# gunrock/mini

Measured on AMD Instinct MI355X. Metric: MTEPS (million traversed edges/sec) BFS advance+filter, RMAT-22, higher is better.
Workload: dtype int32

## Files before the change

### include/mgx/bfs_fused.hpp

```cpp
#pragma once
#include <cstdlib>
#include <cstring>
#include <memory>

#include "runtime.hpp"
#include "env.hpp"
#include "wave.hpp"

namespace mgx {

constexpr int BFS_MAX_TRACE = 4096;
constexpr int BFS_VSHIFT = 38;
constexpr u64 BFS_EMASK = (1ull << BFS_VSHIFT) - 1ull;

struct bfs_ctrl_t {
  u64 cursor[3];
  u64 pad_a_[13];
  u64 lcursor[3];
  u64 pad_b_[13];
  u64 ledges[3];
  u64 pad_c_[13];
  u64 reached;
  u64 pad_d_[15];
  u64 merged_new;
// ... 41 lines not shown

struct bfs_fused_args_t {
  const u32* row_offsets;
  const int* col_indices;
  int* labels;
  u32* visited;
  unsigned char* mark;
  u32* frontier_bits;
  u32* fr_row[2];
  u32* fr_off[2];
  u32* lq_row[2];
  u32* lq_off[2];
  bfs_ctrl_t* ctrl;
  const u32* in_offsets;
  const int* in_indices;
  const int* old_of_new;
  const int* new_of_old;
  int long_min;
  u32 hot_min_edges;
  int mode;
  float alpha;
  int n;
  int count_marks;
  const int* ub_col;
  const u32* ub_col24;
  const int* ub_owner;
  u32 ub_units;
  u32 ub_units_pad;
  u32 ub_hot_only;
  const u32* ubf_col24;
  const int* ubf_owner;
  u32 ubf_units_pad;
  u32 dense_div;
  u32 vs_v[4];
  u32 vs_v9;
  u32 vs_edges;
  u32 vs_div;
  u32 vs_dummy;
  u32* flush_buf;
  u32 defer_min_marks;
  u32 defer_words;
  u32 defer_reach_mul, defer_reach_div;
  int lazy_pull;
  int merged_pull;
  u32 chain_max_edges;
  u32 chain_big_edges;
  u32 lazy_div;
  u32* slot_marks;
  const int* cold_owner;
  const int* cold_dst;
  int cold_slices;
  u32 cold_lo[BFS_COLD_MAX_SLICES];
  u32 cold_off[BFS_COLD_MAX_SLICES + 1];
  u32 cold_wgs[BFS_COLD_MAX_SLICES + 1];
  u32* cold_flush;
  u32 cold_all = 0;
  u64 cold_all_pairs = 0;
  const u32* cold_pk = nullptr;
  const u32* cold_cbase = nullptr;
  u64 cold_pk_mask = 0;
  u32 cold_ranks = 1;
  u32 cold_cb[BFS_COLD_MAX_SLICES + 1] = {};
  u32* d2_list = nullptr;
  u32 d2_list_cap = 0;
  u32* d2_newbits = nullptr;
  u32* d2_front = nullptr;
  const int* vs_col = nullptr;
  const int* colds_owner = nullptr;
  const int* colds_dst = nullptr;
  u32 colds_off[BFS_COLD_MAX_SLICES + 1] = {};
#ifdef MGX_LAB
  int flags;
  int build_diag;
  int dense_diag;
#endif
};

#ifdef MGX_LAB
#define MGX_LAB_GET(obj, field, product_value) ((obj).field)
#else
#define MGX_LAB_GET(obj, field, product_value) (product_value)
#endif

template <int NT, int WORDS>
__device__ __forceinline__ void bfs_copy_prefix(u32* __restrict__ dst, const u32* __restrict__ src) {
  static_assert(WORDS % 4 == 0, "whole 16-byte pieces");
  constexpr int Q = WORDS / 4;
  constexpr int IT = (Q + NT - 1) / NT;
  const uint4* const s4 = (const uint4*)src;
  uint4* const d4 = (uint4*)dst;
  uint4 v[IT];
#pragma unroll
  for (int k = 0; k < IT; ++k) {
    const int i = k * NT + (int)threadIdx.x;
    v[k] = s4[i < Q ? i : Q - 1];
  }
#pragma unroll
  for (int k = 0; k < IT; ++k) {
    const int i = k * NT + (int)threadIdx.x;
    if (i < Q) d4[i] = v[k];
  }
}

constexpr int BFS_COLD_WGS = 64;
constexpr int BFS_COLD_WGS_MAX = 1024;
constexpr int BFS_COLD_WORDS = 20384;

constexpr int BFS_MARK_CTRS = 8;
constexpr int BFS_MARK_STRIDE = 32;

__device__ __forceinline__ void bfs_body_finish(const bfs_fused_args_t& a, int marks, int slot, int stat_level, int* s_int) {
  if (!a.slot_marks && !a.count_marks) return;
  marks = wave_sum(marks);
  if ((threadIdx.x & (WAVE - 1)) == 0 && marks) atomicAdd(&s_int[0], marks);
  __syncthreads();
  if (threadIdx.x == 0 && s_int[0]) {
    if (a.slot_marks) atomicAdd(&a.slot_marks[((slot & 1) * BFS_MARK_CTRS + (int)(blockIdx.x % BFS_MARK_CTRS)) * BFS_MARK_STRIDE], (u32)s_int[0]);
    if (a.count_marks) {
      atomicAdd(&a.ctrl->claims, (u64)s_int[0]);
      if (stat_level < 64) atomicAdd(&a.ctrl->claims_level[stat_level], (u64)s_int[0]);
    }
  }
}
__device__ __forceinline__ void bfs_slot_marks_clear(const bfs_fused_args_t& a, int slot) {
  if (a.slot_marks)
    for (int i = 0; i < BFS_MARK_CTRS; ++i) a.slot_marks[((slot & 1) * BFS_MARK_CTRS + i) * BFS_MARK_STRIDE] = 0u;
}

__device__ __forceinline__ void bfs_ctrl_reset(bfs_ctrl_t* c) {
  for (int i = 0; i < 3; ++i) { c->cursor[i] = 0; c->lcursor[i] = 0; c->ledges[i] = 0; }
  c->merged_new = 0;
  c->sum_edges = c->sum_frontier = c->sum_long_edges = c->sum_long_vertices = 0;
  c->reached = 1;
  c->claims = 0;
  for (int i = 0; i < 64; ++i) c->claims_level[i] = 0;
  c->pull_edges = 0;
  c->done = c->levels = c->pull = c->push_levels = 0;
  c->d2_append_level = c->d2_declared_level = -1;
  c->small_levels = c->slots = 0;
  c->dist_done = c->dist_levels = 0;
  for (int i = 0; i < 4; ++i) { c->slot_level[i] = 0; c->skip_build[i] = 0; }
  c->flush_count[0] = c->flush_count[1] = 0;
  c->fb_slot = 0;
  c->dense_slots = 0;
  c->vshort_slots = 0;
  c->lazy_slot = -1;
  c->lazy_slots = 0;
  c->cold_slot = -1;
  c->cold_slots = 0;
  c->mini_slots = 0;
  for (int i = 0; i < 4; ++i) c->mini_blocks[i] = 0u;
  c->reached_mini = 0;
  c->d2_frozen_level = -1;
  for (int i = 0; i < 16; ++i) ((u32*)c->d2_level_kind)[i] = 0u;
  for (int i = 0; i < 64; ++i) c->d2_level_new[i] = 0u;
  c->sssp_thr = 0x7f7fffffu;
  c->sssp_far_cnt[0] = c->sssp_far_cnt[1] = 0;
  c->sssp_far_min[0] = c->sssp_far_min[1] = 0x7f7fffffu;
  for (int i = 0; i < 64; ++i) c->stamp[i] = 0;
}

__host__ __device__ __forceinline__ u32 bfs_lq_pad(u32 deg) { return (deg + 63u) & ~63u; }
__host__ __device__ __forceinline__ u32 bfs_lq_degree(u32 entry, u32 next_entry) {
  return ((next_entry & ~63u) - (entry & ~63u)) - ((64u - (entry & 63u)) & 63u);
}

__device__ __forceinline__ void bfs_seed_queue(const bfs_fused_args_t& a, u32 row) {
  bfs_ctrl_t* c = a.ctrl;
  const u32 ro = a.row_offsets[row];
  const u32 deg = a.row_offsets[row + 1] - ro;
  const bool is_long = a.long_min > 0 && deg >= (u32)a.long_min;
  (is_long ? a.lq_row : a.fr_row)[0][0] = ro;
  (is_long ? a.lq_off : a.fr_off)[0][0] = is_long ? (deg & 63u) : 0u;
  (is_long ? c->lcursor : c->cursor)[0] = deg ? ((1ull << BFS_VSHIFT) | (u64)(is_long ? bfs_lq_pad(deg) : deg)) : 0ull;
  if (is_long) c->ledges[0] = deg;
}

template <int NT>
__device__ __forceinline__ void bfs_init_body(const bfs_fused_args_t& a, int src, long long nwords, const bfs_ctrl_t* prev_ctrl,
                                              bfs_ctrl_t* prev_head, int head_words, u32 blk, u32 nblk) {
  if (prev_head && blk == 0) {
    const u32* const from = (const u32*)prev_ctrl;
    u32* const to = (u32*)prev_head;
    for (int i = threadIdx.x; i < head_words; i += NT) to[i] = from[i];
    __syncthreads();
  }
  const int src_old = src;
  if (a.new_of_old) src = a.new_of_old[src];
  const long long tid = (long long)blk * NT + threadIdx.x;
  const long long nth = (long long)nblk * NT;
  const long long n = a.n;
  for (long long i = tid; i < (n + 3) / 4; i += nth) {
    if (i * 4 + 4 <= n) {
      const long long j = i * 4;
      const int4 l = make_int4(src_old == j ? 0 : -1, src_old == j + 1 ? 0 : -1, src_old == j + 2 ? 0 : -1,
                               src_old == j + 3 ? 0 : -1);
      *(int4*)(a.labels + j) = l;
      *(u32*)(a.mark + i * 4) = 0u;
    } else {
      for (long long j = i * 4; j < n; ++j) { a.labels[j] = (j == src_old) ? 0 : -1; a.mark[j] = 0; }
    }
  }
  const u32 src_bit = 1u << (src & 31);
  for (long long w = tid; w < nwords; w += nth) {
    const u32 seed = (w == (src >> 5)) ? src_bit : 0u;
    a.visited[w] = seed;
    a.frontier_bits[w] = seed;
  }
  if (tid == 0) {
    bfs_ctrl_reset(a.ctrl);
    bfs_slot_marks_clear(a, 0);
    bfs_slot_marks_clear(a, 1);
    bfs_seed_queue(a, (u32)src);
  }
}
__global__ __launch_bounds__(BLOCK) void k_bfs_fused_init(bfs_fused_args_t a, int src, long long nwords, const bfs_ctrl_t* prev_ctrl,
                                                          bfs_ctrl_t* prev_head, int head_words) {
  bfs_init_body<BLOCK>(a, src, nwords, prev_ctrl, prev_head, head_words, blockIdx.x, gridDim.x);
}

__device__ __forceinline__ bool bfs_open_level(const bfs_fused_args_t& a, int level, int slot) {
  bfs_ctrl_t* const c = a.ctrl;
  const u64 cur = c->cursor[slot % 3];
  const u64 lcur = c->lcursor[slot % 3];
  const long long nf = (long long)(cur >> BFS_VSHIFT) + (long long)(lcur >> BFS_VSHIFT);
  const u64 long_edges = c->ledges[slot % 3];
  const u64 E = (cur & BFS_EMASK) + long_edges;
  c->cursor[(slot + 2) % 3] = 0;
  c->lcursor[(slot + 2) % 3] = 0;
  c->ledges[(slot + 2) % 3] = 0;
  if (level < 64) c->stamp[level] = __builtin_amdgcn_s_memrealtime();
  if (nf == 0) {
    if (!c->done) { c->done = 1; c->levels = level; }
    return false;
  }
  if (level < BFS_MAX_TRACE) c->trace[level] = ((u64)nf << BFS_VSHIFT) | E;
  c->sum_edges += E;
  c->sum_frontier += (u64)nf;
  c->sum_long_edges += long_edges;
  c->sum_long_vertices += lcur >> BFS_VSHIFT;
  if (a.mode == 1 && !c->pull) {
    const float unvisited = (float)((long long)a.n - (long long)c->reached);
    if (unvisited < (float)nf * a.alpha) c->pull = 1;
  }
  if (!c->pull) c->push_levels += 1;
  return true;
}

__device__ __forceinline__ bool bfs_level_pulls(const bfs_fused_args_t& a, const bfs_ctrl_t* c, int slot) {
  if (a.mode != 1) return false;
  if (c->pull) return true;
  const long long nf = (long long)(c->cursor[slot % 3] >> BFS_VSHIFT) + (long long)(c->lcursor[slot % 3] >> BFS_VSHIFT);
  const float unvisited = (float)((long long)a.n - (long long)c->reached);
  return unvisited < (float)nf * a.alpha;
}

__device__ __forceinline__ void bfs_begin_level(const bfs_fused_args_t& a, int level, int partitioned) {
  bfs_ctrl_t* const c = a.ctrl;
  if (partitioned && level > 0 && c->merged_new == 0 && !c->dist_done) { c->dist_done = 1; c->dist_levels = level; }
  (void)bfs_open_level(a, level, level);
}
__global__ void k_bfs_level_begin(bfs_fused_args_t a, int level, int partitioned) {
  if (blockIdx.x != 0 || threadIdx.x != 0) return;
  bfs_begin_level(a, level, partitioned);
}

__device__ __forceinline__ bool bfs_d2_frozen(const bfs_ctrl_t* c, int level) {
  const int f = c->d2_frozen_level;
  return f >= 0 && level > f;
}

__device__ __forceinline__ void bfs_resolve(const bfs_ctrl_t* c, int arg, int& slot, int& level) {
  if (arg >= 0) { slot = level = arg; return; }
  slot = -1 - arg;
  level = c->slot_level[slot & 3];
}
__host__ __device__ __forceinline__ int bfs_slot_arg(int slot) { return -1 - slot; }

constexpr int BFS_FLUSH_WORDS = 20352;
constexpr int BFS_FLUSH_MAX = 1024;
constexpr int BFS_FLUSH_RUNS = BFS_FLUSH_WORDS / 32;

__device__ __forceinline__ u32 bfs_defer_limit(const bfs_fused_args_t& a, u32 hot_n) {
  if (!a.flush_buf || hot_n == 0u) return 0u;
  const u32 range = hot_n < a.defer_words * 32u ? hot_n : a.defer_words * 32u;
  return a.ctrl->reached * (u64)a.defer_reach_mul < (u64)range * (u64)a.defer_reach_div ? range : 0u;
}

template <int NT>
__device__ __forceinline__ int bfs_hot_epilogue(const bfs_fused_args_t& a, const u32* hot, u32 defer_words, int slot,
                                                int* s_red, int marks) {
  if (defer_words == 0u) return 0;
  constexpr int PERT = (BFS_FLUSH_WORDS + NT - 1) / NT;
  if (threadIdx.x == 0) { s_red[0] = 0; s_red[1] = -1; }
  __syncthreads();
  const int wm = wave_sum(marks);
  if (lane_id() == 0 && wm) atomicAdd(&s_red[0], wm);
  __syncthreads();
  const int total = s_red[0];
  if (total == 0) return 0;
  if (MGX_LAB_GET(a, dense_diag, 0) & 8) return total;
  if ((u32)total > a.defer_min_marks) {
    if (threadIdx.x == 0) {
      const u32 k = atomicAdd(&a.ctrl->flush_count[slot & 1], 1u);
      s_red[1] = k < (u32)BFS_FLUSH_MAX ? (int)k : -1;
    }
    __syncthreads();
    const int k = s_red[1];
    if (k >= 0) {
      u32* const out = a.flush_buf + (size_t)k * BFS_FLUSH_WORDS;
#pragma unroll
      for (int q = 0; q < PERT; ++q) {
        const u32 i = (u32)q * NT + threadIdx.x;
        if (i < a.defer_words) out[i] = i < defer_words ? hot[i] : 0u;
      }
      return total;
    }
  }
  constexpr int CH = 5;
#pragma unroll
  for (int q0 = 0; q0 < PERT; q0 += CH) {
    u32 vis[CH];
#pragma unroll
    for (int k = 0; k < CH; ++k) {
      const u32 i = (u32)(q0 + k) * NT + threadIdx.x;
      vis[k] = __hip_atomic_load(a.visited + (i < defer_words ? i : 0u), __ATOMIC_RELAXED, __HIP_MEMORY_SCOPE_WAVEFRONT);
    }
#pragma unroll
    for (int k = 0; k < CH; ++k) {
      if (q0 + k >= PERT) break;
      const u32 i = (u32)(q0 + k) * NT + threadIdx.x;
      u32 w = i < defer_words ? (hot[i] & ~vis[k]) : 0u;
      const u32 base = i * 32u;
      while (w) {
        const int b = __ffs((int)w) - 1;
        w &= w - 1u;
        a.mark[base + (u32)b] = 1;
      }
    }
  }
  return total;
}

struct __attribute__((aligned(4))) bfs_u32x2 { u32 x, y; };

constexpr int BFS_BUILD_NT = 1024;
constexpr int BFS_BUILD_VPB = 16 * BFS_BUILD_NT;
constexpr int BFS_BUILD_LIST = 8 * BFS_BUILD_NT;

inline int bfs_build_grid(long long n_local, int nt = BFS_BUILD_NT) { return (int)((n_local + 16 * nt - 1) / (16 * nt)); }

template <int NT, bool FROM_MARKS>
__global__ __launch_bounds__(NT, NT == 512 ? 4 : 4) void k_bfs_build(bfs_fused_args_t a, int arg, const u32* __restrict__ bits,
                                                  int* __restrict__ labels, int n_local, int ranks, int rank,
                                                  int stop_when_done) {
  constexpr int NW = NT / WAVE;
  constexpr int LIST = 8 * NT;
  constexpr int PER = LIST / NT;
  constexpr u64 CNT1 = 1ull << 40;
  constexpr u64 DEGMASK = CNT1 - 1ull;
  __shared__ u32 st_v[LIST];
  __shared__ u32 st_d[LIST];
  __shared__ u64 s_scan[NW + 1];
  __shared__ u64 s_base[2];
  __shared__ u32 s_long_edges;
  bfs_ctrl_t* const c = a.ctrl;
  int slot, level;
  bfs_resolve(c, arg, slot, level);
  if (stop_when_done && c->done) return;
  if (!FROM_MARKS && bfs_d2_frozen(c, level)) return;
  if (arg < 0 && c->skip_build[slot & 3]) return;
  if (FROM_MARKS && blockIdx.x == 0 && threadIdx.x == 0) c->fb_slot = slot + 1;
  const long long i0 = (((long long)blockIdx.x + (long long)(threadIdx.x >> 6) * gridDim.x) * 64 + (threadIdx.x & 63)) * 16;
  const int new_label = level + 1;
  const int* __restrict__ old_of_new = a.old_of_new;
  const u32 long_min = a.long_min > 0 ? (u32)a.long_min : 0xFFFFFFFFu;

  u32 flushed16 = 0;
  if (FROM_MARKS && a.flush_buf) {
    const u32 F = (MGX_LAB_GET(a, build_diag, 0) & 32) ? 0u : c->flush_count[slot & 1];
    if (F) {
      __shared__ u32 s_or[NW][WAVE];
      const int wave = threadIdx.x >> 6, lane = threadIdx.x & 63;
      for (int hr = 0; hr < NW; ++hr) {
        const long long run = (long long)blockIdx.x + (long long)hr * gridDim.x;
        if (run >= (long long)(a.defer_words / 32u)) break;
        const unsigned short* const col = (const unsigned short*)a.flush_buf + run * 64 + lane;
        u32 acc = 0;
#pragma unroll 16
        for (u32 k = (u32)wave; k < F; k += NW) acc |= col[(size_t)k * (BFS_FLUSH_WORDS * 2)];
        s_or[wave][lane] = acc;
        __syncthreads();
        if (wave == hr) {
#pragma unroll
          for (int w = 0; w < NW; ++w) flushed16 |= s_or[w][lane];
        }
        __syncthreads();
      }
    }
  }

  u32 new16 = 0;
  if (i0 < n_local) {
    const u32 valid = (n_local - i0 >= 16) ? 0xFFFFu : ((1u << (int)(n_local - i0)) - 1u);
    if (FROM_MARKS) {
      const uint4 m = *(const uint4*)(a.mark + i0);
      const u32 x[4] = {m.x, m.y, m.z, m.w};
      u32 m16 = 0;
#pragma unroll
      for (int q = 0; q < 4; ++q) m16 |= (((x[q] & 0x01010101u) * 0x10204080u) >> 28) << (4 * q);
      m16 |= flushed16;
      unsigned short* const vis16 = (unsigned short*)a.visited + (i0 >> 4);
      const u32 old16 = *vis16;
      new16 = m16 & ~old16 & valid;
      if (new16) *vis16 = (unsigned short)(old16 | new16);
      ((unsigned short*)a.frontier_bits)[i0 >> 4] = (unsigned short)new16;
    } else {
      for (int q = 0; q < 16; ++q) {
        const long long v = (i0 + q) * ranks + rank;
        if (((valid >> q) & 1u) && ((bits[v >> 5] >> (v & 31)) & 1u)) new16 |= 1u << q;
      }
    }
  }
  u64 total64;
  const u64 before = block_exclusive_sum_lean<NW>((u64)__popc(new16), s_scan, &total64);
  const int total = (int)total64;
  if (total == 0) return;
  if (threadIdx.x == 0) atomicAdd(&c->reached, (u64)total);

  u64* const cur_s = &c->cursor[(slot + 1) % 3];
  u64* const cur_l = &c->lcursor[(slot + 1) % 3];
  u32* __restrict__ const out_row_s = a.fr_row[(slot + 1) & 1];
  u32* __restrict__ const out_off_s = a.fr_off[(slot + 1) & 1];
  u32* __restrict__ const out_row_l = a.lq_row[(slot + 1) & 1];
  u32* __restrict__ const out_off_l = a.lq_off[(slot + 1) & 1];

  for (int first = 0; first < total; first += LIST) {
    {
      u32 rest = new16;
      int at = (int)before - first;
      while (rest) {
        const int q = __ffs((int)rest) - 1;
        rest &= rest - 1;
        if (at >= 0 && at < LIST) st_v[at] = (u32)(i0 + q);
        ++at;
      }
    }
    if (threadIdx.x == 0) s_long_edges = 0;
    __syncthreads();
    const int cnt = (total - first < LIST) ? total - first : LIST;
#pragma unroll
    for (int q = 0; q < PER; ++q) {
      const int i = q * NT + threadIdx.x;
      if (i < cnt) {
        const u32 v = st_v[i];
        bfs_u32x2 ext;
        if (MGX_LAB_GET(a, build_diag, 0) & 2) { ext.x = v * 8u; ext.y = v * 8u + 3u; }
        else ext = *(const bfs_u32x2*)(a.row_offsets + v);
        if (!(MGX_LAB_GET(a, build_diag, 0) & 1)) labels[old_of_new ? old_of_new[v] : (int)v] = new_label;
        st_v[i] = ext.x;
        st_d[i] = ext.y - ext.x;
      }
    }
    __syncthreads();
    u32 ro[PER], dg[PER];
#pragma unroll
    for (int q = 0; q < PER; ++q) {
      const int i = threadIdx.x * PER + q;
      ro[q] = (i < cnt) ? st_v[i] : 0u;
      dg[q] = (i < cnt) ? st_d[i] : 0u;
    }
    u64 loc[PER];
    u64 sum_s = 0, sum_l = 0;
    u32 longmask = 0, long_true = 0;
#pragma unroll
    for (int q = 0; q < PER; ++q) {
      const u32 deg = dg[q];
      const bool is_long = deg >= long_min;
      if (is_long) { longmask |= 1u << q; long_true += deg; }
      loc[q] = is_long ? sum_l : sum_s;
      const u64 add = deg ? (CNT1 | (u64)(is_long ? bfs_lq_pad(deg) : deg)) : 0ull;
      if (is_long) sum_l += add; else sum_s += add;
    }
    long_true = wave_sum(long_true);
    if ((threadIdx.x & (WAVE - 1)) == 0 && long_true) atomicAdd(&s_long_edges, long_true);
    u64 tot_s, tot_l;
    const u64 ex_s = block_exclusive_sum_lean<NW>(sum_s, s_scan, &tot_s);
    const u64 ex_l = block_exclusive_sum_lean<NW>(sum_l, s_scan, &tot_l);
    if (threadIdx.x == 0) {
      if (MGX_LAB_GET(a, build_diag, 0) & 4) { s_base[0] = ((u64)blockIdx.x * 4096) << BFS_VSHIFT; s_base[1] = ((u64)blockIdx.x * 4096) << BFS_VSHIFT; }
      else {
      s_base[0] = (tot_s >> 40) ? atomicAdd(cur_s, ((tot_s >> 40) << BFS_VSHIFT) | (tot_s & DEGMASK)) : 0ull;
      s_base[1] = (tot_l >> 40) ? atomicAdd(cur_l, ((tot_l >> 40) << BFS_VSHIFT) | (tot_l & DEGMASK)) : 0ull;
      }
      if (tot_l >> 40) atomicAdd(&c->ledges[(slot + 1) % 3], (u64)s_long_edges);
    }
    __syncthreads();
#pragma unroll
    for (int q = 0; q < PER; ++q) {
      if (dg[q] != 0u) {
        const bool is_long = (longmask >> q) & 1u;
        const u64 base = is_long ? s_base[1] : s_base[0];
        const u64 at = (is_long ? ex_l : ex_s) + loc[q];
        const u64 slot = (base >> BFS_VSHIFT) + (at >> 40);
        (is_long ? out_row_l : out_row_s)[slot] = ro[q];
        (is_long ? out_off_l : out_off_s)[slot] =
            (u32)((base & BFS_EMASK) + (at & DEGMASK)) | (is_long ? (dg[q] & 63u) : 0u);
      }
    }
    __syncthreads();
  }
}

__device__ __forceinline__ bool bfs_build_is_lazy(const bfs_fused_args_t& a, int slot) {
  if (a.lazy_div == 0u || !a.slot_marks) return false;
  u64 M = 0;
#pragma unroll
  for (int i = 0; i < BFS_MARK_CTRS; ++i) M += a.slot_marks[((slot & 1) * BFS_MARK_CTRS + i) * BFS_MARK_STRIDE];
  return M * (u64)a.lazy_div >= (u64)(u32)a.n;
}

struct bfs_d2_fuse_t {
  const u32* maps = nullptr;
  int nmaps = 0;
  long long stride = 0;
  long long nwords = 0;
  u32* merged = nullptr;
  u32* clear = nullptr;
  u32* list_head = nullptr;
};
template <int NT, int DIST = 0, int RANKS = 1>
__global__ __launch_bounds__(NT, 4) void k_bfs_build2(bfs_fused_args_t a, int arg, int* __restrict__ labels, int n,
                                                      const u32* __restrict__ bits = nullptr, int ranks = 1, int rank = 0,
                                                      bfs_d2_fuse_t fz = bfs_d2_fuse_t()) {
  constexpr int NW = NT / WAVE;
  constexpr u64 CNT1 = 1ull << 40;
  constexpr u64 DEGMASK = CNT1 - 1ull;
  __shared__ u64 s_scan[NW + 1];
  __shared__ u64 s_base[2];
  __shared__ u32 s_long_edges;
  __shared__ u32 s_or[NW][WAVE];
  bfs_ctrl_t* const c = a.ctrl;
  uint4 pre_m = make_uint4(0u, 0u, 0u, 0u);
  u32 pre_old16 = 0u;
  if (!DIST) {
    const long long j0 = ((((long long)blockIdx.x + (long long)(threadIdx.x % NW) * gridDim.x) * 64 + (threadIdx.x / NW)) * 16);
    const long long jc = j0 < (long long)n ? j0 : 0;
    pre_m = *(const uint4*)(a.mark + jc);
    pre_old16 = ((const unsigned short*)a.visited)[jc >> 4];
  }
  int slot, level;
  bfs_resolve(c, arg, slot, level);
  if (!DIST && (c->done || c->skip_build[slot & 3])) return;
  if (DIST && bfs_d2_frozen(c, level)) return;
  if (DIST == 2 && fz.list_head && blockIdx.x == 0 && threadIdx.x == 0) fz.list_head[0] = 0u;
  const bool lazy = !DIST && (bfs_build_is_lazy(a, slot) || (a.lazy_pull && c->pull));
  if (!DIST && blockIdx.x == 0 && threadIdx.x == 0) {
    c->fb_slot = slot + 1;
    c->lazy_slot = lazy ? slot + 1 : -1;
    if (lazy) c->lazy_slots += 1;
  }
  const int wave = threadIdx.x >> 6, lane = threadIdx.x & 63;
  const int my_run = threadIdx.x % NW, my_group = threadIdx.x / NW;
  const long long i0 = (((long long)blockIdx.x + (long long)my_run * gridDim.x) * 64 + my_group) * 16;
  const int new_label = level + 1;
  const u32 long_min = a.long_min > 0 ? (u32)a.long_min : 0xFFFFFFFFu;

  u32 flushed16 = 0;
  if (!DIST && a.flush_buf) {
    const u32 F = (MGX_LAB_GET(a, build_diag, 0) & 32) ? 0u : c->flush_count[slot & 1];
    if (F) {
      for (int hr = 0; hr < NW; ++hr) {
        const long long run = (long long)blockIdx.x + (long long)hr * gridDim.x;
        if (run >= (long long)(a.defer_words / 32u)) break;
        const uint4* const base = (const uint4*)(a.flush_buf + (size_t)run * 32) + (lane & 7);
        uint4 acc = make_uint4(0u, 0u, 0u, 0u);
#pragma unroll 8
        for (u32 k = (u32)wave * 8u + ((u32)lane >> 3); k < F; k += 8u * NW) {
          const uint4 v = base[(size_t)k * (BFS_FLUSH_WORDS / 4)];
          acc.x |= v.x; acc.y |= v.y; acc.z |= v.z; acc.w |= v.w;
        }
#pragma unroll
        for (int sh = 8; sh < 64; sh <<= 1) {
          acc.x |= __shfl_xor(acc.x, sh, WAVE); acc.y |= __shfl_xor(acc.y, sh, WAVE);
          acc.z |= __shfl_xor(acc.z, sh, WAVE); acc.w |= __shfl_xor(acc.w, sh, WAVE);
        }
        if (lane < 8) *(uint4*)(&s_or[wave][lane * 4]) = acc;
        __syncthreads();
        if (my_run == hr) {
#pragma unroll
          for (int w = 0; w < NW; ++w) flushed16 |= (u32)((const unsigned short*)&s_or[w][0])[my_group];
        }
        __syncthreads();
      }
    }
  }

  if (!DIST && a.cold_dst && c->cold_slot == slot && !(MGX_LAB_GET(a, build_diag, 0) & 64)) {
    static_assert(NW == 8, "one wave per run");
    u32* const s_run = &s_or[0][0];
    const long long run = (long long)blockIdx.x + (long long)wave * gridDim.x;
    const long long v0 = run * 1024;
    int sl = -1;
    for (int q = 0; q < a.cold_slices; ++q)
      if (v0 >= (long long)a.cold_lo[q] && v0 < (long long)a.cold_lo[q] + (long long)BFS_COLD_WORDS * 32) sl = q;
    uint4 acc = make_uint4(0u, 0u, 0u, 0u);
    if (sl >= 0) {
      const u32 rel = (u32)((v0 - (long long)a.cold_lo[sl]) >> 10);
// ... 413 lines not shown
```

### include/mgx/bfs_fused_chain.hpp

```cpp
#pragma once
#include "bfs_fused.hpp"

namespace mgx {

constexpr int BFS_CHAIN_NT = 1024;
constexpr int BFS_CHAIN_CAP = 6144;
constexpr int BFS_CHAIN_EPT = 4;
constexpr int BFS_CHAIN_CAP_BIG = 12288;
constexpr size_t bfs_chain_lds_bytes(int cap = BFS_CHAIN_CAP) {
  return (size_t)(BFS_CHAIN_NT / 64 + 2) * 8 + (size_t)(3 * cap + 4) * 4 + 64;
}

constexpr u32 BFS_CHAIN_EARLY_EDGES = 1536;
__device__ __forceinline__ bool bfs_rule_pulls(const bfs_fused_args_t& a, u64 reached, u64 nf) {
  const float unvisited = (float)((long long)a.n - (long long)reached);
  return unvisited < (float)(long long)nf * a.alpha;
}
__device__ __forceinline__ u32 bfs_chain_edge_limit(const bfs_fused_args_t& a, u64 reached, u32 max_edges) {
  const bool late = reached * 4ull >= (u64)(u32)a.n;
  return late || max_edges < BFS_CHAIN_EARLY_EDGES ? max_edges : BFS_CHAIN_EARLY_EDGES;
}
__device__ __forceinline__ bool bfs_level_is_chained(const bfs_fused_args_t& a, u64 cur, u64 lcur, u64 ledges, u32 max_edges, int list_cap = BFS_CHAIN_CAP) {
  if (max_edges == 0u) return false;
  const u64 nf = (cur >> BFS_VSHIFT) + (lcur >> BFS_VSHIFT);
  const u64 E = (cur & BFS_EMASK) + ledges;
  if (a.mode == 1 && (a.ctrl->pull || bfs_rule_pulls(a, a.ctrl->reached, nf))) return false;
  const u32 lim = bfs_chain_edge_limit(a, a.ctrl->reached, max_edges);
  const u64 cap = lim < (u32)list_cap ? lim : (u32)list_cap;
  return nf <= (u64)list_cap && E <= cap;
}
__device__ __forceinline__ bool bfs_level_is_chained(const bfs_fused_args_t& a, u64 cur, u64 lcur, u64 ledges) {
  return bfs_level_is_chained(a, cur, lcur, ledges, a.chain_max_edges);
}

template <int NT, bool INPLACE = false, int CAP = BFS_CHAIN_CAP>
__device__ __forceinline__ void bfs_chain_body(const bfs_fused_args_t& a, int slot, int level) {
  constexpr int NW = NT / WAVE;
  constexpr int EPT = BFS_CHAIN_EPT;
  constexpr u64 CNT1 = 1ull << 40;
  constexpr u64 DEGMASK = CNT1 - 1ull;
  static_assert(CAP % NT == 0, "chain list shape");
  extern __shared__ __attribute__((aligned(16))) char smem[];
  u64* const s_scan = (u64*)smem;
  u32* const s_off = (u32*)(s_scan + NW + 2);
  u32* const s_row = s_off + CAP + 2;
  u32* const s_win = s_row + CAP;
  int* const s_i = (int*)(s_win + CAP);
  bfs_ctrl_t* const c = a.ctrl;
  const int lane = lane_id();
  const u32 long_min = a.long_min > 0 ? (u32)a.long_min : 0xFFFFFFFFu;
  const u32 lim_e = INPLACE ? a.chain_big_edges : a.chain_max_edges;

  int nf;
  u32 E;
  {
    const u64 cur = c->cursor[slot % 3], lcur = c->lcursor[slot % 3];
    const int nf_l = (int)(lcur >> BFS_VSHIFT), nf_s = (int)(cur >> BFS_VSHIFT);
    const u32 El = (u32)(lcur & BFS_EMASK), Es = (u32)(cur & BFS_EMASK);
    const u32* __restrict__ lq_row = a.lq_row[slot & 1];
    const u32* __restrict__ lq_off = a.lq_off[slot & 1];
    const u32* __restrict__ fr_row = a.fr_row[slot & 1];
    const u32* __restrict__ fr_off = a.fr_off[slot & 1];
    nf = nf_l + nf_s;
    u64 run = 0;
    for (int first = 0; first < nf; first += NT) {
      const int i = first + threadIdx.x;
      u32 row = 0, deg = 0;
      if (i < nf_l) {
        const u32 e0 = lq_off[i], e1 = (i + 1 < nf_l) ? lq_off[i + 1] : El;
        row = lq_row[i];
        deg = bfs_lq_degree(e0, e1);
      } else if (i < nf) {
        const int j = i - nf_l;
        const u32 e0 = fr_off[j], e1 = (j + 1 < nf_s) ? fr_off[j + 1] : Es;
        row = fr_row[j];
        deg = e1 - e0;
      }
      u64 tot;
      const u64 ex = run + block_exclusive_sum_lean<NW>((u64)deg, s_scan, &tot);
      if (i < nf) { s_row[i] = row; s_off[i] = (u32)ex; }
      run += tot;
    }
    E = (u32)run;
    if (threadIdx.x == 0) s_off[nf] = E;
  }

  for (int chained = 0;; ++chained) {
    if (threadIdx.x == 0) {
      if (level < 64) c->stamp[level] = __builtin_amdgcn_s_memrealtime();
      if (level < BFS_MAX_TRACE) c->trace[level] = ((u64)nf << BFS_VSHIFT) | (u64)E;
      c->sum_edges += (u64)E;
      c->sum_frontier += (u64)nf;
      c->push_levels += 1;
      c->small_levels += 1;
      if (chained == 0 && !INPLACE) c->slots += 1;
      s_i[0] = 0;
    }
    __syncthreads();

    {
      int top = 1;
      while (top * 2 < nf) top *= 2;
      for (u32 base = 0; base < E; base += NT * EPT) {
        u32 r[EPT];
        int sj[EPT];
        bool act[EPT];
#pragma unroll
        for (int k = 0; k < EPT; ++k) {
          r[k] = base + (u32)(k * NT) + threadIdx.x;
          act[k] = r[k] < E;
          if (!act[k]) r[k] = 0;
          sj[k] = 0;
        }
        if (nf > 1)
          for (int step = top; step > 0; step >>= 1) {
#pragma unroll
            for (int k = 0; k < EPT; ++k) {
              const int j = sj[k] + step;
              if (j < nf && s_off[j] <= r[k]) sj[k] = j;
            }
          }
        int d[EPT];
#pragma unroll
        for (int k = 0; k < EPT; ++k) d[k] = a.col_indices[act[k] ? s_row[sj[k]] + (r[k] - s_off[sj[k]]) : 0u];
        u32 seen[EPT];
#pragma unroll
        for (int k = 0; k < EPT; ++k) seen[k] = act[k] ? a.visited[(u32)d[k] >> 5] : 0xFFFFFFFFu;
        u32 old[EPT];
#pragma unroll
        for (int k = 0; k < EPT; ++k) {
          const u32 bit = 1u << (d[k] & 31);
          old[k] = (seen[k] & bit) ? 0xFFFFFFFFu : atomicOr(a.visited + ((u32)d[k] >> 5), bit);
        }
#pragma unroll
        for (int k = 0; k < EPT; ++k) {
          const bool win = !(old[k] & (1u << (d[k] & 31)));
          const u64 bal = __ballot(win);
          if (bal) {
            int at = 0;
            if (lane == 0) at = atomicAdd(&s_i[0], __popcll(bal));
            at = __builtin_amdgcn_readfirstlane(at);
            if (win) s_win[at + rank_in_mask(bal)] = (u32)d[k];
          }
        }
      }
    }
    __syncthreads();

    const int W = s_i[0];
    const int new_label = level + 1;
    u64 run = 0;
    constexpr int WPT = 4;
    for (int first = 0; first < W; first += WPT * NT) {
      u32 ro[WPT], dg[WPT];
      u64 mine = 0;
#pragma unroll
      for (int q = 0; q < WPT; ++q) {
        const int i = first + threadIdx.x * WPT + q;
        ro[q] = 0; dg[q] = 0;
        if (i < W) {
          const u32 v = s_win[i];
          const bfs_u32x2 ext = *(const bfs_u32x2*)(a.row_offsets + v);
          ro[q] = ext.x;
          dg[q] = ext.y - ext.x;
          a.labels[a.old_of_new ? a.old_of_new[v] : (int)v] = new_label;
        }
        if (dg[q]) mine += CNT1 | (u64)dg[q];
      }
      u64 tot;
      u64 ex = run + block_exclusive_sum_lean<NW>(mine, s_scan, &tot);
#pragma unroll
      for (int q = 0; q < WPT; ++q) {
        if (dg[q]) {
          s_row[ex >> 40] = ro[q];
          s_off[ex >> 40] = (u32)(ex & DEGMASK);
          ex += CNT1 | (u64)dg[q];
        }
      }
      run += tot;
    }
    const int nf2 = (int)(run >> 40);
    const u32 E2 = (u32)(run & DEGMASK);
    if (threadIdx.x == 0) {
      s_off[nf2] = E2;
      const u64 reached_now = c->reached + (u64)W;
      c->reached = reached_now;
      s_i[1] = (int)bfs_chain_edge_limit(a, reached_now, lim_e);
      s_i[2] = (a.mode == 1 && bfs_rule_pulls(a, reached_now, (u64)nf2)) ? 1 : 0;
      if (a.count_marks) { c->claims += (u64)W; if (level < 64) c->claims_level[level] += (u64)W; }
    }
    __syncthreads();

    const u32 max_l = (u32)s_i[1];
    const u32 max_e = max_l < (u32)CAP ? max_l : (u32)CAP;
    const bool next_pulls = s_i[2] != 0;
    if (nf2 != 0 && (run & DEGMASK) <= (u64)max_e && !next_pulls) {
      nf = nf2;
      E = E2;
      level += 1;
      continue;
    }

    const int out = INPLACE ? slot : slot + 1;
    u32* __restrict__ const out_row_s = a.fr_row[out & 1];
    u32* __restrict__ const out_off_s = a.fr_off[out & 1];
    u32* __restrict__ const out_row_l = a.lq_row[out & 1];
    u32* __restrict__ const out_off_l = a.lq_off[out & 1];
    u64 tot_s = 0, tot_l = 0, tot_true = 0;
    for (int first = 0; first < nf2; first += NT) {
      const int i = first + threadIdx.x;
      u32 ro = 0, dg = 0;
      if (i < nf2) { ro = s_row[i]; dg = s_off[i + 1] - s_off[i]; }
      const bool is_long = dg >= long_min;
      const u64 add_s = (!is_long && dg) ? (CNT1 | (u64)dg) : 0ull;
      const u64 add_l = is_long ? (CNT1 | (u64)bfs_lq_pad(dg)) : 0ull;
      u64 ts, tl, tt;
      const u64 ex_s = tot_s + block_exclusive_sum_lean<NW>(add_s, s_scan, &ts);
      const u64 ex_l = tot_l + block_exclusive_sum_lean<NW>(add_l, s_scan, &tl);
      (void)block_exclusive_sum_lean<NW>(is_long ? (u64)dg : 0ull, s_scan, &tt);
      if (is_long) {
        out_row_l[ex_l >> 40] = ro;
        out_off_l[ex_l >> 40] = (u32)(ex_l & DEGMASK) | (dg & 63u);
      } else if (dg) {
        out_row_s[ex_s >> 40] = ro;
        out_off_s[ex_s >> 40] = (u32)(ex_s & DEGMASK);
      }
      tot_s += ts; tot_l += tl; tot_true += tt;
    }
    if (nf2 != 0 && (next_pulls || (a.ub_owner && a.dense_div && ((tot_l & DEGMASK) >> 6) * (u64)a.dense_div >= (u64)a.ub_units))) {
      uint4* const fb4 = (uint4*)a.frontier_bits;
      const int quads = (a.n + 127) / 128;
      for (int i = threadIdx.x; i < quads; i += NT) fb4[i] = make_uint4(0u, 0u, 0u, 0u);
      __threadfence();
      __syncthreads();
      for (int i = threadIdx.x; i < W; i += NT) {
        const u32 v = s_win[i];
        atomicOr(a.frontier_bits + (v >> 5), 1u << (v & 31u));
      }
      if (threadIdx.x == 0) c->fb_slot = out;
    } else if (INPLACE) {
      if (threadIdx.x == 0) c->fb_slot = -1;
    }
    if (threadIdx.x == 0) {
      c->cursor[out % 3] = ((tot_s >> 40) << BFS_VSHIFT) | (tot_s & DEGMASK);
      c->lcursor[out % 3] = ((tot_l >> 40) << BFS_VSHIFT) | (tot_l & DEGMASK);
      c->ledges[out % 3] = tot_true;
      c->slot_level[out & 3] = level + 1;
      if (!INPLACE) {
        c->cursor[(slot + 2) % 3] = 0;
        c->lcursor[(slot + 2) % 3] = 0;
        c->ledges[(slot + 2) % 3] = 0;
        c->skip_build[slot & 3] = 1;
        c->flush_count[(slot + 1) & 1] = 0;
        bfs_slot_marks_clear(a, slot + 1);
      }
      if (nf2 == 0 && !c->done) { c->done = 1; c->levels = level + 1; }
    }
    return;
  }
}

}
```

### include/mgx/bfs_fused_mini.hpp

```cpp
#pragma once
#include "bfs_fused.hpp"
#include "bfs_fused_chain.hpp"

namespace mgx {

constexpr int BFS_MINI_WGS = 64;
constexpr int BFS_MINI_LCAP = 4096;
constexpr int BFS_MINI_WCAP = 8192;
constexpr u32 BFS_MINI_EDGES_LATE = 131072;
constexpr u32 BFS_MINI_EDGES_EARLY = 32768;
constexpr u32 BFS_MINI_SHORT_ROWS = 65536;
constexpr size_t bfs_mini_lds_bytes() {
  return (size_t)(2 * BFS_MINI_LCAP + 4) * 4 + (size_t)BFS_MINI_WCAP * 4 + 64 * 8 + 256;
}

__device__ __forceinline__ bool bfs_level_is_mini(const bfs_fused_args_t& a, const bfs_ctrl_t* c, int slot) {
  if (a.mode != 0 || c->lazy_slot == slot) return false;
  const u64 cur = c->cursor[slot % 3], lcur = c->lcursor[slot % 3];
  const u64 E = (cur & BFS_EMASK) + c->ledges[slot % 3];
  const bool late = c->reached * 4ull >= (u64)(u32)a.n;
  return (lcur >> BFS_VSHIFT) <= (u64)BFS_MINI_LCAP && (cur >> BFS_VSHIFT) <= (u64)BFS_MINI_SHORT_ROWS &&
         E <= (u64)(late ? BFS_MINI_EDGES_LATE : BFS_MINI_EDGES_EARLY);
}

template <int NT>
__device__ __forceinline__ void bfs_mini_body(const bfs_fused_args_t& a, int arg, u32 blk, u32 nblk) {
  constexpr int NW = NT / WAVE;
  constexpr u64 CNT1 = 1ull << 40;
  constexpr u64 DEGMASK = CNT1 - 1ull;
  extern __shared__ __attribute__((aligned(16))) char smem[];
  u32* const s_loff = (u32*)smem;
  u32* const s_lrow = s_loff + BFS_MINI_LCAP + 4;
  u32* const s_win = s_lrow + BFS_MINI_LCAP;
  u64* const s_scan = (u64*)(s_win + BFS_MINI_WCAP);
  __shared__ int s_cnt, s_maxdeg;
  __shared__ u64 s_base[2];
  __shared__ u32 s_long_true;
  bfs_ctrl_t* const c = a.ctrl;
  int slot, level;
  bfs_resolve(c, arg, slot, level);
  if (c->done) return;
  const u64 cur = c->cursor[slot % 3], lcur = c->lcursor[slot % 3];
  const u64 ledges = c->ledges[slot % 3];
  const int nf_s = (int)(cur >> BFS_VSHIFT), nf_l = (int)(lcur >> BFS_VSHIFT);
  const u32 Es = (u32)(cur & BFS_EMASK), Rl = (u32)(lcur & BFS_EMASK);
  const int in = slot & 1, out = (slot + 1) & 1;
  const bool first_thread = blk == 0 && threadIdx.x == 0;
  if (nf_s + nf_l == 0) {
    if (first_thread) {
      c->cursor[(slot + 2) % 3] = 0; c->lcursor[(slot + 2) % 3] = 0; c->ledges[(slot + 2) % 3] = 0;
      if (level < 64) c->stamp[level] = __builtin_amdgcn_s_memrealtime();
      if (!c->done) { c->done = 1; c->levels = level; }
    }
    return;
  }
  const long long gtid = (long long)blk * NT + threadIdx.x, gthreads = (long long)nblk * NT;
  if (!bfs_level_is_mini(a, c, slot)) {
    const bool lazy = c->lazy_slot == slot;
    const bool fb = c->fb_slot == slot;
    if (!lazy) {
      for (long long i = gtid; i < nf_s; i += gthreads) { a.fr_row[out][i] = a.fr_row[in][i]; a.fr_off[out][i] = a.fr_off[in][i]; }
      for (long long i = gtid; i < nf_l; i += gthreads) { a.lq_row[out][i] = a.lq_row[in][i]; a.lq_off[out][i] = a.lq_off[in][i]; }
    }
    __syncthreads();
    if (threadIdx.x == 0) {
      __threadfence();
      if (atomicAdd(&c->mini_blocks[slot & 3], 1u) == nblk - 1u) {
        c->mini_blocks[slot & 3] = 0u;
        c->cursor[(slot + 1) % 3] = cur; c->lcursor[(slot + 1) % 3] = lcur; c->ledges[(slot + 1) % 3] = ledges;
        c->cursor[(slot + 2) % 3] = 0; c->lcursor[(slot + 2) % 3] = 0; c->ledges[(slot + 2) % 3] = 0;
        c->slot_level[(slot + 1) & 3] = level;
        c->flush_count[(slot + 1) & 1] = 0;
        bfs_slot_marks_clear(a, slot + 1);
        if (lazy) c->lazy_slot = slot + 1;
        if (fb) c->fb_slot = slot + 1;
      }
    }
    return;
  }
  if (first_thread) {
    const u64 E = (u64)Es + ledges;
    c->cursor[(slot + 2) % 3] = 0; c->lcursor[(slot + 2) % 3] = 0; c->ledges[(slot + 2) % 3] = 0;
    if (level < 64) c->stamp[level] = __builtin_amdgcn_s_memrealtime();
    if (level < BFS_MAX_TRACE) c->trace[level] = ((u64)(nf_s + nf_l) << BFS_VSHIFT) | E;
    c->sum_edges += E;
    c->sum_frontier += (u64)(nf_s + nf_l);
    c->sum_long_edges += ledges;
    c->sum_long_vertices += (u64)nf_l;
    c->push_levels += 1;
    c->small_levels += 1;
    c->mini_slots += 1;
    c->slots += 1;
    c->slot_level[(slot + 1) & 3] = level + 1;
    c->flush_count[(slot + 1) & 1] = 0;
    bfs_slot_marks_clear(a, slot + 1);
    c->fb_slot = -1;
  }
  const int lane = lane_id();
  const int wave = threadIdx.x / WAVE;
  const u32 long_min = a.long_min > 0 ? (u32)a.long_min : 0xFFFFFFFFu;
  const int new_label = level + 1;
  for (int i = threadIdx.x; i < nf_l; i += NT) { s_loff[i] = a.lq_off[in][i]; s_lrow[i] = a.lq_row[in][i]; }
  if (threadIdx.x == 0) { s_loff[nf_l] = Rl; s_cnt = 0; s_maxdeg = 0; }
  __syncthreads();

  u64* const cur_s = &c->cursor[(slot + 1) % 3];
  u64* const cur_l = &c->lcursor[(slot + 1) % 3];
  u32* __restrict__ const out_row_s = a.fr_row[out];
  u32* __restrict__ const out_off_s = a.fr_off[out];
  u32* __restrict__ const out_row_l = a.lq_row[out];
  u32* __restrict__ const out_off_l = a.lq_off[out];
  int found = 0;

  auto flush = [&]() {
    __syncthreads();
    const int W = s_cnt;
    for (int first = 0; first < W; first += NT) {
      const int i = first + (int)threadIdx.x;
      u32 ro = 0, deg = 0;
      if (i < W) {
        const u32 v = s_win[i];
        const bfs_u32x2 ext = *(const bfs_u32x2*)(a.row_offsets + v);
        ro = ext.x; deg = ext.y - ext.x;
        a.labels[a.old_of_new ? a.old_of_new[v] : (int)v] = new_label;
      }
      const bool is_long = deg >= long_min;
      const u64 add_s = (!is_long && deg) ? (CNT1 | (u64)deg) : 0ull;
      const u64 add_l = is_long ? (CNT1 | (u64)bfs_lq_pad(deg)) : 0ull;
      if (threadIdx.x == 0) s_long_true = 0;
      u64 tot_s, tot_l;
      const u64 ex_s = block_exclusive_sum_lean<NW>(add_s, s_scan, &tot_s);
      const u64 ex_l = block_exclusive_sum_lean<NW>(add_l, s_scan, &tot_l);
      const u32 lt = wave_sum(is_long ? deg : 0u);
      if (lane == 0 && lt) atomicAdd(&s_long_true, lt);
      __syncthreads();
      if (threadIdx.x == 0) {
        s_base[0] = (tot_s >> 40) ? atomicAdd(cur_s, ((tot_s >> 40) << BFS_VSHIFT) | (tot_s & DEGMASK)) : 0ull;
        s_base[1] = (tot_l >> 40) ? atomicAdd(cur_l, ((tot_l >> 40) << BFS_VSHIFT) | (tot_l & DEGMASK)) : 0ull;
        if (tot_l >> 40) atomicAdd(&c->ledges[(slot + 1) % 3], (u64)s_long_true);
      }
      __syncthreads();
      if (deg) {
        const u64 b = is_long ? s_base[1] : s_base[0];
        const u64 at = is_long ? ex_l : ex_s;
        const u64 pos = (b >> BFS_VSHIFT) + (at >> 40);
        (is_long ? out_row_l : out_row_s)[pos] = ro;
        (is_long ? out_off_l : out_off_s)[pos] = (u32)((b & BFS_EMASK) + (at & DEGMASK)) | (is_long ? (deg & 63u) : 0u);
      }
      __syncthreads();
    }
    if (threadIdx.x == 0) s_cnt = 0;
    __syncthreads();
  };
  auto visit = [&](bool act, u32 d) {
    bool win = false;
    if (act) {
      const u32 bit = 1u << (d & 31u);
      const u32 seen = a.visited[d >> 5];
      if (!(seen & bit)) win = !(atomicOr(a.visited + (d >> 5), bit) & bit);
    }
    const u64 bal = __ballot(win);
    if (bal) {
      int at = 0;
      if (lane == 0) at = atomicAdd(&s_cnt, __popcll(bal));
      at = __builtin_amdgcn_readfirstlane(at);
      if (win) { s_win[at + rank_in_mask(bal)] = d; ++found; }
    }
  };

  {
    const u32 U = Rl >> 6;
    const u32 Wt = nblk * NW, w0 = blk * NW + (u32)wave;
    const u32 iters = (U + Wt - 1u) / Wt;
    for (u32 t = 0; t < iters; ++t) {
      const u32 u = w0 + t * Wt;
      bool act = false;
      u32 d = 0;
      if (u < U) {
        const u32 r0 = u << 6;
        int lo = 0, hi = nf_l;
        while (hi - lo > 1) { const int mid = (lo + hi) >> 1; if ((s_loff[mid] & ~63u) <= r0) lo = mid; else hi = mid; }
        const u32 e0 = s_loff[lo];
        const u32 deg = bfs_lq_degree(e0, s_loff[lo + 1]);
        const u32 rank = r0 - (e0 & ~63u) + (u32)lane;
        act = rank < deg;
        if (act) d = (u32)a.col_indices[s_lrow[lo] + rank];
      }
      visit(act, d);
      __syncthreads();
      const int cnt_now = s_cnt;
      __syncthreads();
      if (cnt_now > BFS_MINI_WCAP - NT) flush();
    }
  }
  if (nf_s > 0 && (u64)Es >= 4ull * (u64)nf_s) {
    const u32* __restrict__ fr_row = a.fr_row[in];
    const u32* __restrict__ fr_off = a.fr_off[in];
    const u32 iters = (Es + (u32)gthreads - 1u) / (u32)gthreads;
    for (u32 t = 0; t < iters; ++t) {
      const u64 r64 = (u64)gtid + (u64)t * (u64)gthreads;
      const bool act = r64 < (u64)Es;
      const u32 r = act ? (u32)r64 : 0u;
      int lo = 0, hi = nf_s;
      while (hi - lo > 1) { const int mid = (lo + hi) >> 1; if (fr_off[mid] <= r) lo = mid; else hi = mid; }
      const u32 d = act ? (u32)a.col_indices[fr_row[lo] + (r - fr_off[lo])] : 0u;
      visit(act, d);
      __syncthreads();
      const int cnt_now = s_cnt;
      __syncthreads();
      if (cnt_now > BFS_MINI_WCAP - NT) flush();
    }
  } else
  {
    const u32* __restrict__ fr_row = a.fr_row[in];
    const u32* __restrict__ fr_off = a.fr_off[in];
    const u32 iters = ((u32)nf_s + (u32)gthreads - 1u) / (u32)gthreads;
    for (u32 t = 0; t < iters; ++t) {
      const long long i = gtid + (long long)t * gthreads;
      u32 row = 0, deg = 0;
      if (i < nf_s) {
        const u32 e0 = fr_off[i], e1 = (i + 1 < nf_s) ? fr_off[i + 1] : Es;
        row = fr_row[i];
        deg = e1 - e0;
      }
      int wmax = (int)deg;
#pragma unroll
      for (int sh = WAVE / 2; sh > 0; sh >>= 1) { const int o = __shfl_xor(wmax, sh, WAVE); wmax = o > wmax ? o : wmax; }
      if (lane == 0 && wmax) atomicMax(&s_maxdeg, wmax);
      __syncthreads();
      const u32 kmax = (u32)s_maxdeg;
      for (u32 k = 0; k < kmax; ++k) {
        const bool act = k < deg;
        const u32 d = act ? (u32)a.col_indices[row + k] : 0u;
        visit(act, d);
        __syncthreads();
        const int cnt_now = s_cnt;
        __syncthreads();
        if (cnt_now > BFS_MINI_WCAP - NT) flush();
      }
      __syncthreads();
      if (threadIdx.x == 0) s_maxdeg = 0;
      __syncthreads();
    }
  }
  flush();
  found = (int)wave_sum((u32)found);
  if (lane == 0 && found) {
    atomicAdd(&c->reached_mini, (u64)found);
    if (a.count_marks) {
      atomicAdd(&c->claims, (u64)found);
      if (level < 64) atomicAdd(&c->claims_level[level], (u64)found);
    }
  }
}
template <int NT>
__global__ __launch_bounds__(NT) void k_bfs_mini(bfs_fused_args_t a, int arg) {
  bfs_mini_body<NT>(a, arg, blockIdx.x, gridDim.x);
}

}
```

Measured before the change: 462,500.

## Keep chained-level counters in registers and split mini-kernel base atomics across waves

In the in-place chain path, thread 0 now keeps the per-level statistics (edges, frontier, reached, level counts) in registers and writes them back to the control block once at exit. This avoids a global read-modify-write on every chained level. The timestamp and trace stores are deferred until after the first gather loads are issued. In the mini kernel, the short-list and long-list cursor atomics now run from two different waves so they can proceed in parallel. A lab-flag path also lets blocks claim flush slots by block index instead of through an atomic counter; it is off by default, and slot collisions with that path are a risk.

```diff
diff --git a/include/mgx/bfs_fused.hpp b/include/mgx/bfs_fused.hpp
--- a/include/mgx/bfs_fused.hpp
+++ b/include/mgx/bfs_fused.hpp
@@ -367,8 +367,13 @@
   if (MGX_LAB_GET(a, dense_diag, 0) & 8) return total;
   if ((u32)total > a.defer_min_marks) {
     if (threadIdx.x == 0) {
+      if (MGX_LAB_GET(a, build_diag, 0) & 128) {
+        s_red[1] = blockIdx.x < (u32)BFS_FLUSH_MAX ? (int)blockIdx.x : -1;
+        if (s_red[1] >= 0) atomicAdd(&a.ctrl->flush_count[slot & 1], 1u);
+      } else {
       const u32 k = atomicAdd(&a.ctrl->flush_count[slot & 1], 1u);
       s_red[1] = k < (u32)BFS_FLUSH_MAX ? (int)k : -1;
+      }
     }
     __syncthreads();
     const int k = s_red[1];
diff --git a/include/mgx/bfs_fused_chain.hpp b/include/mgx/bfs_fused_chain.hpp
--- a/include/mgx/bfs_fused_chain.hpp
+++ b/include/mgx/bfs_fused_chain.hpp
@@ -46,6 +46,8 @@
   u32* const s_row = s_off + CAP + 2;
   u32* const s_win = s_row + CAP;
   int* const s_i = (int*)(s_win + CAP);
+  u64 acc_edges = 0, acc_frontier = 0, acc_reached = 0;
+  int acc_push = 0, acc_small = 0;
   bfs_ctrl_t* const c = a.ctrl;
   const int lane = lane_id();
   const u32 long_min = a.long_min > 0 ? (u32)a.long_min : 0xFFFFFFFFu;
@@ -62,6 +64,10 @@
     const u32* __restrict__ fr_row = a.fr_row[slot & 1];
     const u32* __restrict__ fr_off = a.fr_off[slot & 1];
     nf = nf_l + nf_s;
+    if (INPLACE && threadIdx.x == 0) {
+      acc_edges = c->sum_edges; acc_frontier = c->sum_frontier; acc_reached = c->reached;
+      acc_push = c->push_levels; acc_small = c->small_levels;
+    }
     u64 run = 0;
     for (int first = 0; first < nf; first += NT) {
       const int i = first + threadIdx.x;
@@ -86,14 +92,23 @@
   }
 
   for (int chained = 0;; ++chained) {
+    u64 t_open = 0;
     if (threadIdx.x == 0) {
-      if (level < 64) c->stamp[level] = __builtin_amdgcn_s_memrealtime();
-      if (level < BFS_MAX_TRACE) c->trace[level] = ((u64)nf << BFS_VSHIFT) | (u64)E;
-      c->sum_edges += (u64)E;
-      c->sum_frontier += (u64)nf;
-      c->push_levels += 1;
-      c->small_levels += 1;
-      if (chained == 0 && !INPLACE) c->slots += 1;
+      if (INPLACE) {
+        t_open = __builtin_amdgcn_s_memrealtime();
+        acc_edges += (u64)E;
+        acc_frontier += (u64)nf;
+        acc_push += 1;
+        acc_small += 1;
+      } else {
+        if (level < 64) c->stamp[level] = __builtin_amdgcn_s_memrealtime();
+        if (level < BFS_MAX_TRACE) c->trace[level] = ((u64)nf << BFS_VSHIFT) | (u64)E;
+        c->sum_edges += (u64)E;
+        c->sum_frontier += (u64)nf;
+        c->push_levels += 1;
+        c->small_levels += 1;
+        if (chained == 0) c->slots += 1;
+      }
       s_i[0] = 0;
     }
     __syncthreads();
@@ -123,6 +138,10 @@
         int d[EPT];
 #pragma unroll
         for (int k = 0; k < EPT; ++k) d[k] = a.col_indices[act[k] ? s_row[sj[k]] + (r[k] - s_off[sj[k]]) : 0u];
+        if (INPLACE && base == 0u && threadIdx.x == 0) {
+          if (level < 64) c->stamp[level] = t_open;
+          if (level < BFS_MAX_TRACE) c->trace[level] = ((u64)nf << BFS_VSHIFT) | (u64)E;
+        }
         u32 seen[EPT];
 #pragma unroll
         for (int k = 0; k < EPT; ++k) seen[k] = act[k] ? a.visited[(u32)d[k] >> 5] : 0xFFFFFFFFu;
@@ -183,8 +202,9 @@
     const u32 E2 = (u32)(run & DEGMASK);
     if (threadIdx.x == 0) {
       s_off[nf2] = E2;
-      const u64 reached_now = c->reached + (u64)W;
-      c->reached = reached_now;
+      const u64 reached_now = (INPLACE ? acc_reached : c->reached) + (u64)W;
+      if (INPLACE) acc_reached = reached_now;
+      else c->reached = reached_now;
       s_i[1] = (int)bfs_chain_edge_limit(a, reached_now, lim_e);
       s_i[2] = (a.mode == 1 && bfs_rule_pulls(a, reached_now, (u64)nf2)) ? 1 : 0;
       if (a.count_marks) { c->claims += (u64)W; if (level < 64) c->claims_level[level] += (u64)W; }
@@ -242,6 +262,10 @@
       if (threadIdx.x == 0) c->fb_slot = -1;
     }
     if (threadIdx.x == 0) {
+      if (INPLACE) {
+        c->sum_edges = acc_edges; c->sum_frontier = acc_frontier; c->reached = acc_reached;
+        c->push_levels = acc_push; c->small_levels = acc_small;
+      }
       c->cursor[out % 3] = ((tot_s >> 40) << BFS_VSHIFT) | (tot_s & DEGMASK);
       c->lcursor[out % 3] = ((tot_l >> 40) << BFS_VSHIFT) | (tot_l & DEGMASK);
       c->ledges[out % 3] = tot_true;
diff --git a/include/mgx/bfs_fused_mini.hpp b/include/mgx/bfs_fused_mini.hpp
--- a/include/mgx/bfs_fused_mini.hpp
+++ b/include/mgx/bfs_fused_mini.hpp
@@ -134,8 +134,8 @@
       const u32 lt = wave_sum(is_long ? deg : 0u);
       if (lane == 0 && lt) atomicAdd(&s_long_true, lt);
       __syncthreads();
-      if (threadIdx.x == 0) {
-        s_base[0] = (tot_s >> 40) ? atomicAdd(cur_s, ((tot_s >> 40) << BFS_VSHIFT) | (tot_s & DEGMASK)) : 0ull;
+      if (threadIdx.x == 0) s_base[0] = (tot_s >> 40) ? atomicAdd(cur_s, ((tot_s >> 40) << BFS_VSHIFT) | (tot_s & DEGMASK)) : 0ull;
+      if (threadIdx.x == WAVE) {
         s_base[1] = (tot_l >> 40) ? atomicAdd(cur_l, ((tot_l >> 40) << BFS_VSHIFT) | (tot_l & DEGMASK)) : 0ull;
         if (tot_l >> 40) atomicAdd(&c->ledges[(slot + 1) % 3], (u64)s_long_true);
       }
```

After: 462,900 (median of 4 runs). Within noise of the previous version (+0.1%).
